# RustAudio/lewton

Hardware: NVIDIA H100
Metric: Msamples/s IMDCT+window+OLA, 2048-pt long blocks (higher is better)
Workload: dtype f32

## Files before the change

include/lewton_b200.h:

```cpp
#ifndef LEWTON_B200_H
#define LEWTON_B200_H

#include <stddef.h>
#include <stdint.h>

#ifdef __cplusplus
extern "C" {
#endif

#define LWB_ABI_VERSION 3
#define LWB_MAX_POSTS 65
#define LWB_MAX_CHANNELS 255
#define LWB_MAX_COUPLING 256
#define LWB_MAX_SUBMAPS 16
#define LWB_MAX_MODES 64

enum {
    LWB_OK = 0,
    LWB_ERR_BAD_FORMAT = 1,
    LWB_ERR_BUFFER = 2,
    LWB_ERR_MISMATCH = 3,
    LWB_ERR_INVALID = 4,
    LWB_ERR_CUDA = 5,
    LWB_ERR_NO_DEVICE = 6
};

typedef struct lwb_ctx lwb_ctx;
typedef struct lwb_setup lwb_setup;
typedef struct lwb_stream lwb_stream;

int lwb_abi_version(void);
int lwb_device_count(void);
int lwb_ctx_create(int device_ordinal, lwb_ctx **out);
void lwb_ctx_destroy(lwb_ctx *ctx);
int lwb_ctx_synchronize(lwb_ctx *ctx);
const char *lwb_last_error(const lwb_ctx *ctx);
void *lwb_ctx_cuda_stream(lwb_ctx *ctx);
uint64_t lwb_ctx_launch_count(const lwb_ctx *ctx);
enum { LWB_KERNEL_LONG = 0, LWB_KERNEL_LONG_S = 1, LWB_KERNEL_MID = 2, LWB_KERNEL_SHORT = 3, LWB_KERNEL_SHORT_G = 4,
       LWB_KERNEL_ROW_COPY = 5, LWB_KERNEL_CHAIN = 6, LWB_KERNEL_FLOOR1_SEGMENTS = 7, LWB_KERNEL_PROLOGUE_FUSED = 8,
       LWB_KERNEL_PROLOGUE = 9, LWB_KERNEL_IMDCT = 10, LWB_KERNEL_OVERLAP = 11, LWB_KERNEL_SAVE_STATE = 12,
       LWB_KERNEL_COUNT = 13 };
uint64_t lwb_ctx_kernel_launches(const lwb_ctx *ctx, int kernel_id);
void *lwb_host_alloc(size_t bytes);
void lwb_host_free(void *p);
int lwb_bind_host_to_device(int device_ordinal);
int lwb_device_alloc(lwb_ctx *ctx, size_t bytes, void **out);
void lwb_device_free(lwb_ctx *ctx, void *p);
int lwb_memcpy_h2d(lwb_ctx *ctx, void *dst_dev, const void *src_host, size_t bytes);
int lwb_memcpy_d2h(lwb_ctx *ctx, void *dst_host, const void *src_dev, size_t bytes);

int lwb_tables_generate(int blocksize_log2, float *a, float *b, float *c, float *window,
                        uint32_t *bitrev);

typedef struct lwb_tables_ref {
    const float *a, *b, *c;
    const float *window;
    const uint32_t *bitrev;
} lwb_tables_ref;

enum { LWB_FLOOR_TYPE_ZERO = 0, LWB_FLOOR_TYPE_ONE = 1 };
typedef struct lwb_floor_desc {
    uint8_t floor_type;
    uint8_t floor1_multiplier;
    uint8_t floor1_values;
    uint8_t reserved;
    uint32_t floor1_x_list[LWB_MAX_POSTS];
} lwb_floor_desc;

typedef struct lwb_mapping_desc {
    uint16_t coupling_steps;
    uint8_t submaps;
    uint8_t reserved;
    uint8_t magnitudes[LWB_MAX_COUPLING];
    uint8_t angles[LWB_MAX_COUPLING];
// ... 139 lines not shown
```

lewton_b200/_cabi.py:

```python
import ctypes as C
import os

_HERE = os.path.dirname(os.path.abspath(__file__))
SO_PATH = os.environ.get("LWB_LIB") or os.path.join(_HERE, "liblewton_b200.so")

MAX_POSTS, MAX_CHANNELS, MAX_COUPLING, MAX_SUBMAPS, MAX_MODES = 65, 255, 256, 16, 64
OK, ERR_BAD_FORMAT, ERR_BUFFER, ERR_MISMATCH, ERR_INVALID, ERR_CUDA, ERR_NO_DEVICE = range(7)
FLOOR_TYPE_ZERO, FLOOR_TYPE_ONE = 0, 1
FLOOR_UNUSED, FLOOR_ONE, FLOOR_DENSE = 0, 1, 2
OUT_F32_PLANAR, OUT_I16_PLANAR, OUT_F32_INTERLEAVED, OUT_I16_INTERLEAVED = 0, 1, 2, 3
ENTRY_SPECTRUM, ENTRY_RESIDUE, ENTRY_VQ = 0, 1, 2
MEM_HOST, MEM_DEVICE = 0, 1
KERNELS = ("k_long", "k_long_s", "k_mid", "k_short", "k_short_g", "k_row_copy", "k_chain", "k_floor1_segments",
           "k_prologue_fused", "k_prologue", "k_imdct", "k_overlap", "k_save_state")

vp, u8p, fp, u32p = C.c_void_p, C.POINTER(C.c_uint8), C.POINTER(C.c_float), C.POINTER(C.c_uint32)


class TablesRef(C.Structure):
    _fields_ = [("a", fp), ("b", fp), ("c", fp), ("window", fp), ("bitrev", u32p)]


class FloorDesc(C.Structure):
    _fields_ = [("floor_type", C.c_uint8), ("floor1_multiplier", C.c_uint8), ("floor1_values", C.c_uint8),
                ("reserved", C.c_uint8), ("floor1_x_list", C.c_uint32 * MAX_POSTS)]


class MappingDesc(C.Structure):
    _fields_ = [("coupling_steps", C.c_uint16), ("submaps", C.c_uint8), ("reserved", C.c_uint8),
                ("magnitudes", C.c_uint8 * MAX_COUPLING), ("angles", C.c_uint8 * MAX_COUPLING),
                ("mux", C.c_uint8 * (MAX_CHANNELS + 1)), ("submap_floors", C.c_uint8 * MAX_SUBMAPS)]


class ModeDesc(C.Structure):
    _fields_ = [("blockflag", C.c_uint8), ("mapping", C.c_uint8)]


class CodebookDesc(C.Structure):
    _fields_ = [("dimensions", C.c_uint16), ("reserved", C.c_uint16), ("entries", C.c_uint32), ("vq", fp)]


class ResidueDesc(C.Structure):
    _fields_ = [("residue_type", C.c_uint8), ("reserved", C.c_uint8 * 3), ("partition_size", C.c_uint32)]


class VqRun(C.Structure):
    _fields_ = [("pos", C.c_uint16), ("first", C.c_uint16), ("book", C.c_uint8), ("pass_kind", C.c_uint8), ("aux", C.c_uint8),
# ... 89 lines not shown
```

lewton_b200/csrc/host_objects.cuh:

```cuda
#pragma once

struct DevBuf {
    void *p = nullptr;
    size_t cap = 0;
};

struct Staging {
    void *h = nullptr;
    size_t cap = 0;
    cudaEvent_t ev = nullptr;
    bool pending = false;
};

struct CachedTables {
    DevTables dt;
    std::vector<float> a, b, c, w;
    std::vector<uint32_t> br;
    std::vector<void *> allocs;
};

struct lwb_ctx {
    int device = 0;
    int sm_count = 0;
    cudaStream_t stream = nullptr;
    cudaStream_t copy_in = nullptr, copy_out = nullptr;
    cudaEvent_t ev_in[64] = {}, ev_done[65] = {};
    DevBuf runs_buf[2];
    cudaEvent_t ev_desc[2] = {}, ev_kdone[2] = {};
    int runs_par = 0;
    uint32_t ticket_next = 0;
    uint64_t epoch = 0;
    uint64_t state_gen = 1;
    std::string err;
    uint64_t launches = 0;
    uint64_t kernel_launches[LWB_KERNEL_COUNT] = {};
    std::vector<PcmSpan> pcm_spans;
    std::vector<PcmCopy> pcm_copies;
    std::deque<CachedTables> tables;
    DevBuf coeffs, dense, pcm, spec, segtab, vqoff, vqrec, magic, x, desc, kinds, ys, chains, ticket, cdesc, cbytes;
    Staging stage[3];
    int stage_next = 0;
    void *h_desc = nullptr;
    size_t h_desc_cap = 0;
    size_t x_cap_elems = (size_t)64 << 20;
};

struct lwb_setup {
    lwb_ctx *ctx = nullptr;
    DevSetup host;
    DevSetup *d_setup = nullptr;
    std::vector<void *> allocs;
    uint8_t channels = 0, bs0 = 0, bs1 = 0;
    uint32_t n_modes = 0;
    uint32_t n_mappings = 0;
    std::vector<DevMapping> mappings;
};

struct MixRound { size_t r0, nr, s0, ns, c0, nc, x0, nx, g0, ng, flat, nm; };
struct RowCopy { const float *src; float *dst; uint32_t n4, pad; };
struct MixLaunch {
    char *db; size_t off_sr, off_cd, off_by, off_rc, off_sg;
    const float *pack, *spack, *w_short, *mpack; int ls, mid_kb; bool i16, residue; int out_format; unsigned warps; size_t smem; int n1max, wpc, np;
    const float *coeffs, *dense; const uint8_t *kinds; const uint32_t *ys; void *pcm;
};

struct FrontStages {
    const DevPacket *pk = nullptr;
    size_t n = 0;
    unsigned C = 0;
    bool fast = false;
    size_t smem_old = 0;
    int n2max = 0;
    uint64_t c_lo = 0;
    uint64_t r_lo = 0, r_hi = 0;
    bool dense = false;
};

struct lwb_plan {
    lwb_ctx *ctx = nullptr;
    lwb_chain *chains = nullptr;
    size_t n_chains = 0;
    lwb_batch_io io;
    bool captured = false;
    uint64_t gen = 0;
    FrontStages front;
    DevBuf runs, pro, mix;
    uint32_t n_groups = 0;
    const float *pack = nullptr;
    bool i16 = false;
    MixLaunch mix_launch;
    std::vector<MixRound> mix_rounds;
};

struct lwb_stream {
    lwb_ctx *ctx = nullptr;
    const lwb_setup *setup = nullptr;
    float *d_state = nullptr;
    bool has = false;
    uint32_t plen = 0;
    uint64_t busy_epoch = 0;
};

static inline void set_stream_state(lwb_stream *s, bool has, uint32_t plen)
{
    if (s->has != has || s->plen != plen) {
        s->has = has;
        s->plen = plen;
        s->ctx->state_gen++;
    }
}

static int fail(lwb_ctx *ctx, int code, const char *what, cudaError_t e = cudaSuccess)
{
    if (ctx) {
        ctx->err = what;
        if (e != cudaSuccess) {
            ctx->err += ": ";
            ctx->err += cudaGetErrorString(e);
        }
    }
    return code;
}

static inline void count_launch(lwb_ctx *ctx, int kernel_id)
{
    ctx->launches++;
    ctx->kernel_launches[kernel_id]++;
}

#define CU(ctx, call)                                                        \
    do {                                                                     \
        cudaError_t e__ = (call);                                            \
        if (e__ != cudaSuccess) return fail((ctx), LWB_ERR_CUDA, #call, e__); \
    } while (0)

static int ensure(lwb_ctx *ctx, DevBuf &b, size_t bytes)
{
    if (bytes <= b.cap) return LWB_OK;
    if (b.p) {
        CU(ctx, cudaStreamSynchronize(ctx->stream));
// ... 117 lines not shown
```

lewton_b200/csrc/kernel_long.cuh:

```cuda
#pragma once
#include <stdint.h>

#if defined(__CUDACC__)
#include <cuda_runtime.h>
#define LWB_HD __host__ __device__ __forceinline__
#else
#define LWB_HD inline
#endif

namespace lwb {

constexpr int kLongBs = 11;
constexpr int kLongN = 2048;
constexpr int kLongN2 = 1024;

struct alignas(16) LongRun {
    const float *in;
    void *out;
    float *state;
    uint32_t in_stride;
    uint32_t n_packets;
    uint8_t has_prev;
    uint8_t write_state;
    uint8_t dummy;
    uint8_t first_short;
    uint8_t last_short;
    uint8_t pad[3];
    float *state_out;
};
static_assert(sizeof(LongRun) == 48, "LongRun is copied by TMA in 16-byte units");

struct V { float x, y; };

#if defined(__CUDA_ARCH__)
__device__ __forceinline__ V vadd(V a, V b) { return V{__fadd_rn(a.x, b.x), __fadd_rn(a.y, b.y)}; }
__device__ __forceinline__ V vsub(V a, V b) { return V{__fsub_rn(a.x, b.x), __fsub_rn(a.y, b.y)}; }
__device__ __forceinline__ V vmul(V a, V b) { return V{__fmul_rn(a.x, b.x), __fmul_rn(a.y, b.y)}; }
__device__ __forceinline__ V vadd_p(V a, V b) { return V{__fadd_rn(a.x, b.x), __fadd_rn(a.y, b.y)}; }
__device__ __forceinline__ V vsub_p(V a, V b) { return V{__fsub_rn(a.x, b.x), __fsub_rn(a.y, b.y)}; }
__device__ __forceinline__ V vnsub_p(V a, V b) { return V{__fsub_rn(-a.x, b.x), __fsub_rn(-a.y, b.y)}; }
#else
inline V vadd(V a, V b) { return V{a.x + b.x, a.y + b.y}; }
inline V vsub(V a, V b) { return V{a.x - b.x, a.y - b.y}; }
inline V vmul(V a, V b) { return V{a.x * b.x, a.y * b.y}; }
inline V vadd_p(V a, V b) { return vadd(a, b); }
inline V vsub_p(V a, V b) { return vsub(a, b); }
inline V vnsub_p(V a, V b) { return V{-a.x - b.x, -a.y - b.y}; }
#endif

enum {
    P_S0W0 = 0, P_S0W1 = 8,
    P_S2W0 = 16, P_S2W1 = 20,
    P_L0W0 = 24, P_L0W1 = 26,
    P_L1W0 = 28, P_L1W1 = 29,
    P_A_END = 30,
    P_L2W0 = 30, P_L2W1 = 34,
    P_L3W0 = 38, P_L3W1 = 40,
    P_L4W0 = 42, P_L4W1 = 43,
    P_B_END = 44,
    P_A2 = 44,
// ... 315 lines not shown
constexpr int kLongWarps = LWB_LONG_WARPS;
constexpr int kLongRing = LWB_LONG_RING;
constexpr int kLongTileBytes = kLongN2 * 4;
constexpr int kLongStageBytes = kLongNB * kLongTileBytes;
constexpr size_t kLongSmemBytes = 2048 + (size_t)kLongWarps * (kLongRing + 1) * kLongStageBytes +
                                  (size_t)kLongPackFloats * 4 + kLongWarps * (kLongRing + 2) * 8 +
                                  kLongWarps * kLongNB * sizeof(LongRun) + 64;

__device__ __forceinline__ uint32_t smem_u32(const void *p) { return (uint32_t)__cvta_generic_to_shared(p); }

__device__ __forceinline__ void mbar_init(uint32_t bar, uint32_t count)
{
    asm volatile("mbarrier.init.shared::cta.b64 [%0], %1;" ::"r"(bar), "r"(count));
}
__device__ __forceinline__ void mbar_expect_tx(uint32_t bar, uint32_t bytes)
{
    asm volatile("mbarrier.arrive.expect_tx.shared::cta.b64 _, [%0], %1;" ::"r"(bar), "r"(bytes) : "memory");
}
__device__ __forceinline__ void mbar_wait(uint32_t bar, uint32_t parity)
{
    asm volatile(
        "{\n\t.reg .pred p;\n\t"
        "WAIT_%=:\n\t"
        "mbarrier.try_wait.parity.shared::cta.b64 p, [%0], %1, %2;\n\t"
        "@p bra DONE_%=;\n\t"
        "bra WAIT_%=;\n\t"
        "DONE_%=:\n\t}" ::"r"(bar), "r"(parity), "r"(200000u) : "memory");
}
__device__ __forceinline__ void tma_load_1d(uint32_t dst, const void *src, uint32_t bytes, uint32_t bar)
{
    asm volatile("cp.async.bulk.shared::cluster.global.mbarrier::complete_tx::bytes [%0], [%1], %2, [%3];"
                 ::"r"(dst), "l"(src), "r"(bytes), "r"(bar) : "memory");
}
__device__ __forceinline__ void fence_proxy_async()
{
    asm volatile("fence.proxy.async.shared::cta;" ::: "memory");
}
__device__ __forceinline__ void sts_eo(uint32_t addr, float e, float o)
{
    asm volatile("st.shared.f32 [%0], %1;\n\tst.shared.f32 [%0+2048], %2;" ::"r"(addr), "f"(e), "f"(o) : "memory");
}
__device__ __forceinline__ void lds_eo(uint32_t addr, float &e, float &o)
{
    asm volatile("ld.shared.f32 %0, [%2];\n\tld.shared.f32 %1, [%2+2048];" : "=f"(e), "=f"(o) : "r"(addr) : "memory");
}

#ifndef LWB_TW_REG0
#define LWB_TW_REG0 0
#endif
#ifndef LWB_TW_REG1
#define LWB_TW_REG1 (LWB_LONG_NB == 2 ? 0 : 53)
#endif
constexpr int kTwReg0 = LWB_TW_REG0;
constexpr int kTwReg1 = LWB_TW_REG1;
struct TwMix {
    const V *r;
    const V *lane_base;
    __device__ __forceinline__ V operator()(int slot) const
    {
        return (slot >= kTwReg0 && slot < kTwReg1) ? r[slot - kTwReg0] : lane_base[slot * 32];
    }
};

__device__ __forceinline__ uint32_t laneA(int lane, int half) { return 4u * (uint32_t)swz(elemA(lane, 0, half)); }
__device__ __forceinline__ uint32_t laneB(int lane) { return 4u * (uint32_t)swz(elemB(lane, 0, 0)); }
__device__ __forceinline__ uint32_t laneC(int lane, int half) { return 4u * (uint32_t)swz(elemC(lane, 0, half)); }
#define LWB_KA(j) (4u * (uint32_t)swz(64 * (j)))
#define LWB_KB(j, h) (4u * (uint32_t)swz(((h) << 6) | ((j) << 3)))
#define LWB_KC(j) (4u * (uint32_t)swz(j))

struct RunCur {
    const float *in;
    void *out;
    float *state;
    uint32_t in_stride;
    uint32_t flags;
};
__device__ __forceinline__ RunCur run_cur(const LongRun &r)
{
    return RunCur{r.in, r.out, r.state, r.in_stride,
                  (uint32_t)(r.has_prev ? 1u : 0u) | (r.write_state ? 2u : 0u) | (r.dummy ? 4u : 0u) |
                      (r.first_short ? 8u : 0u) | (r.last_short ? 16u : 0u)};
}
struct RunCurS : RunCur { float *state_out; };
__device__ __forceinline__ RunCurS run_cur_s(const LongRun &r)
{
    RunCurS c;
    static_cast<RunCur &>(c) = run_cur(r);
    c.flags |= r.first_short == 2 ? 32u : 0u;
    c.state_out = r.state_out ? r.state_out : r.state;
    return c;
}

__device__ __forceinline__ int16_t d_sample_i16(float v)
{
    short r;
    asm("cvt.rzi.s16.f32 %0, %1;" : "=h"(r) : "f"(__fmul_rn(v, 32768.0f)));
    return (int16_t)r;
}
__device__ __forceinline__ void st_pcm(float *p, float v) { __stcs(p, v); }
__device__ __forceinline__ void st_pcm(int16_t *p, float v) { __stcs(reinterpret_cast<short *>(p), (short)d_sample_i16(v)); }

template <int NB, bool FIRST, typename OutT, typename RC = RunCur>
__device__ __forceinline__ void out_stage(const TwMix &tw, int lane, const V O[NB][8], const V E[NB][8], V pe[NB][8],
                                          const RC cur[NB], OutT *out[NB], const float *s_state)
{
#pragma unroll
    for (int j = 0; j < 8; j++) {
        const int r64 = 64 * rev3(j);
        const bool nat = (j & 1);
        const V b0 = tw(P_B0 + j), b1 = tw(P_B1 + j);
        const V wlo = tw(P_WLO + j), whi = tw(P_WHI + j);
#pragma unroll
        for (int b = 0; b < NB; b++) {
            V plo = pe[b][j], phi = pe[b][j];
            bool emit = !(cur[b].flags & 4u);
            if (FIRST) {
                emit = emit && (cur[b].flags & 1u);
                if (cur[b].flags & 1u) {
                    const float *s_lo = s_state + b * kLongN2 + lane, *s_hi = s_state + b * kLongN2 + 63 - lane;
                    const float ax = nat ? s_lo[r64] : s_hi[r64], ay = nat ? s_hi[r64] : s_lo[r64];
                    const float bx = nat ? s_hi[960 - r64] : s_lo[960 - r64];
                    const float by = nat ? s_lo[960 - r64] : s_hi[960 - r64];
                    plo = V{ax, ay};
                    phi = V{bx, by};
                }
            }
            V lo, hi, pev;
            step8_ola(b0, b1, wlo, whi, O[b][j], E[b][j], plo, phi, lo, hi, pev);
            pe[b][j] = pev;
            if (emit) {
                OutT *o_lo = out[b] + lane, *o_hi = out[b] + 63 - lane;
                if (nat) {
                    st_pcm(o_lo + r64, lo.x); st_pcm(o_hi + r64, lo.y);
                    st_pcm(o_hi + 960 - r64, hi.x); st_pcm(o_lo + 960 - r64, hi.y);
                } else {
                    st_pcm(o_hi + r64, lo.x); st_pcm(o_lo + r64, lo.y);
                    st_pcm(o_lo + 960 - r64, hi.x); st_pcm(o_hi + 960 - r64, hi.y);
                }
            }
        }
    }
}

__device__ __forceinline__ float lds_f32(uint32_t addr)
{
    float v;
    asm volatile("ld.shared.f32 %0, [%1];" : "=f"(v) : "r"(addr) : "memory");
    return v;
}

template <int NB, typename OutT, typename RC = RunCur, bool EXPORT = false, int LS = 0>
__device__ __forceinline__ void out_first_short(const TwMix &tw, int lane, const V O[NB][8], const V E[NB][8], V pe[NB][8],
                                                const RC cur[NB], OutT *out[NB], const float *s_state,
                                                const float *__restrict__ w, int ls_arg, uint32_t w_s = 0)
{
    const int ls = LS ? LS : ls_arg;
    const int pl = kLongN2 - 2 * ls;
// ... 77 lines not shown
    const uint32_t bar_state = bars_s + 8 * kLongRing, bar_desc = bars_s + 8 * (kLongRing + 1);
    const uint32_t state_s = smem_u32(s_state), next_s = smem_u32(s_next);
    const uint32_t lA0 = laneA(lane, 0), lA1 = laneA(lane, 1);
    const uint32_t lB = laneB(lane);
    const uint32_t lC0 = laneC(lane, 0), lC1 = laneC(lane, 1);
    uint32_t phase_bits = 0;
    uint32_t slot_i = 0;

    uint32_t lc = 0;
    uint32_t nx_idx = 0;
    uint32_t nx_stage = 0;
    uint32_t nx_lc = 0, nx_npk = 0;
    uint32_t nx_state_issued = 0;
    uint32_t desc_parity = 0;
    RunCur cur[NB];
    uint32_t npk;

    auto issue_stage = [&](uint32_t stage, const LongRun *r, uint32_t pkt) {
        const uint32_t bar = bars_s + 8 * stage;
        mbar_expect_tx(bar, kLongStageBytes);
#pragma unroll
        for (int b = 0; b < NB; b++)
            tma_load_1d(tiles_s + stage * kLongStageBytes + b * kLongTileBytes,
                        r[b].in + (size_t)pkt * r[b].in_stride, kLongTileBytes, bar);
    };
    auto issue_stage_cur = [&](uint32_t stage, uint32_t pkt) {
        const uint32_t bar = bars_s + 8 * stage;
        mbar_expect_tx(bar, kLongStageBytes);
#pragma unroll
        for (int b = 0; b < NB; b++)
            tma_load_1d(tiles_s + stage * kLongStageBytes + b * kLongTileBytes,
                        cur[b].in + (size_t)pkt * cur[b].in_stride, kLongTileBytes, bar);
    };
    auto issue_state = [&](const float *const st[NB], const uint32_t has[NB]) {
        uint32_t bytes = 0;
#pragma unroll
        for (int b = 0; b < NB; b++) bytes += has[b] ? kLongTileBytes : 0;
        mbar_expect_tx(bar_state, bytes);
#pragma unroll
        for (int b = 0; b < NB; b++)
            if (has[b]) tma_load_1d(state_s + b * kLongTileBytes, st[b], kLongTileBytes, bar_state);
    };

    {
        uint32_t idx = 0;
        if (lane == 0) idx = atomicAdd(ticket, 1u);
        idx = __shfl_sync(0xffffffffu, idx, 0);
        if (idx >= n_groups) return;
#pragma unroll
        for (int b = 0; b < NB; b++) cur[b] = run_cur(runs[idx * NB + b]);
        npk = runs[idx * NB].n_packets;
        if (lane == 0) {
            fence_proxy_async();
            const float *st[NB];
            uint32_t has[NB];
#pragma unroll
            for (int b = 0; b < NB; b++) { st[b] = cur[b].state; has[b] = cur[b].flags & 1u; }
            issue_state(st, has);
            for (; lc < (uint32_t)kLongRing && lc < npk; lc++) issue_stage_cur(lc, lc);
            nx_idx = atomicAdd(ticket, 1u);
        }
    }

    for (;;) {
        V pe[NB][8];
#pragma unroll
        for (int b = 0; b < NB; b++)
#pragma unroll
            for (int j = 0; j < 8; j++) pe[b][j] = V{0.f, 0.f};
        OutT *out[NB];
#pragma unroll
        for (int b = 0; b < NB; b++) out[b] = static_cast<OutT *>(cur[b].out);

        for (uint32_t p = 0; p < npk; p++) {
            const uint32_t stage_s = tiles_s + slot_i * kLongStageBytes;
            mbar_wait(bars_s + 8 * slot_i, (phase_bits >> slot_i) & 1u);
            phase_bits ^= 1u << slot_i;

            V O[NB][8], E[NB][8];
            {
                const float *tp[NB];
#pragma unroll
                for (int b = 0; b < NB; b++) tp[b] = tiles + (slot_i * NB + b) * kLongN2;
                phase_a<NB>(tp, lane, tw, O, E);
            }
            __syncwarp();
#pragma unroll
            for (int b = 0; b < NB; b++) {
                const uint32_t t = stage_s + b * kLongTileBytes;
                const uint32_t a0 = t + lA0, a1 = t + lA1;
#pragma unroll
// ... 49 lines not shown
                uint32_t ahead = lc - (p + 1) + nx_lc;
                if (ahead < (uint32_t)kLongRing) {
                    uint32_t tgt = slot_i + 1 + ahead;
                    if (tgt >= (uint32_t)kLongRing) tgt -= kLongRing;
                    if (lc < npk) {
                        fence_proxy_async();
                        issue_stage_cur(tgt, lc);
                        lc++;
                    } else {
                        if (nx_stage == 1) {
                            mbar_wait(bar_desc, desc_parity);
                            desc_parity ^= 1u;
                            nx_stage = 2;
                            nx_npk = s_next[0].n_packets;
                            nx_lc = 0;
                        }
                        if (nx_stage == 2 && nx_lc < nx_npk) {
                            fence_proxy_async();
                            issue_stage(tgt, s_next, nx_lc);
                            nx_lc++;
                        }
                    }
                }
            }
            phase_c_fft<NB>(tw, O, E);
            if (p > 0) {
                out_stage<NB, false, OutT>(tw, lane, O, E, pe, cur, out, s_state);
            } else {
                mbar_wait(bar_state, (phase_bits >> 30) & 1u);
                phase_bits ^= 1u << 30;
                if (NB == 1 && (cur[0].flags & 8u))
                    out_first_short<NB, OutT>(tw, lane, O, E, pe, cur, out, s_state, w_short, ls);
                else
                    out_stage<NB, true, OutT>(tw, lane, O, E, pe, cur, out, s_state);
                __syncwarp();
            }
#pragma unroll
            for (int b = 0; b < NB; b++)
                if (p > 0 || (cur[b].flags & 1u)) out[b] += (p == 0 && (cur[b].flags & 8u)) ? kLongN2 - ls : kLongN2;
            if (lane == 0 && nx_stage == 2 && !nx_state_issued) {
                const float *st[NB];
                uint32_t has[NB];
#pragma unroll
                for (int b = 0; b < NB; b++) { st[b] = s_next[b].state; has[b] = s_next[b].has_prev; }
                fence_proxy_async();
                issue_state(st, has);
                nx_state_issued = 1;
            }
            slot_i = (slot_i + 1 == (uint32_t)kLongRing) ? 0 : slot_i + 1;
        }
#pragma unroll
        for (int b = 0; b < NB; b++) {
            if ((cur[b].flags & 16u)) {
                const bool emitted = (npk > 1 || (cur[b].flags & 1u)) && !(cur[b].flags & 4u);
                const bool keep = (cur[b].flags & 6u) == 2u;
#pragma unroll
                for (int j = 0; j < 8; j++) {
                    const int r64 = 64 * rev3(j);
#pragma unroll
                    for (int h = 0; h < 2; h++) {
                        const float v = ((j & 1) != 0) == (h == 0) ? pe[b][j].x : pe[b][j].y;
                        const int m = r64 + (h ? 63 - lane : lane);
                        if (m < ls) {
                            if (emitted) st_pcm(out[b] + m, v);
                        } else if (keep && m < kLongN2 - ls) {
                            cur[b].state[m - ls] = v;
                            cur[b].state[kLongN2 - 1 - ls - m] = v;
                        }
                    }
                }
            } else if ((cur[b].flags & 6u) == 2u) {
                float *s_lo = cur[b].state + lane, *s_hi = cur[b].state + 63 - lane;
#pragma unroll
                for (int j = 0; j < 8; j++) {
                    const int r64 = 64 * rev3(j);
                    const float vx = (j & 1) ? pe[b][j].x : pe[b][j].y, vy = (j & 1) ? pe[b][j].y : pe[b][j].x;
                    s_lo[r64] = vx; s_hi[r64] = vy;
                    s_hi[960 - r64] = vx; s_lo[960 - r64] = vy;
                }
            }
        }
        uint32_t st_ = 0, nlc = 0;
        if (lane == 0) {
            if (nx_stage == 0) {
                if (nx_idx < n_groups) {
                    fence_proxy_async();
                    mbar_expect_tx(bar_desc, NB * (uint32_t)sizeof(LongRun));
                    tma_load_1d(next_s, runs + (size_t)nx_idx * NB, NB * (uint32_t)sizeof(LongRun), bar_desc);
                    nx_stage = 1;
                } else {
                    nx_stage = 3;
                }
            }
            if (nx_stage == 1) {
                mbar_wait(bar_desc, desc_parity);
                desc_parity ^= 1u;
                nx_stage = 2;
                nx_npk = s_next[0].n_packets;
                nx_lc = 0;
            }
            if (nx_stage == 2 && !nx_state_issued) {
                const float *st[NB];
                uint32_t has[NB];
#pragma unroll
                for (int b = 0; b < NB; b++) { st[b] = s_next[b].state; has[b] = s_next[b].has_prev; }
                fence_proxy_async();
                issue_state(st, has);
            }
            st_ = nx_stage;
            nlc = nx_lc;
        }
        st_ = __shfl_sync(0xffffffffu, st_, 0);
        nlc = __shfl_sync(0xffffffffu, nlc, 0);
        if (st_ != 2) break;
        __syncwarp();
#pragma unroll
        for (int b = 0; b < NB; b++) cur[b] = run_cur(s_next[b]);
        npk = s_next[0].n_packets;
        __syncwarp();
        lc = nlc;
        nx_stage = 0; nx_lc = 0; nx_npk = 0; nx_state_issued = 0;
        if (lane == 0) {
            fence_proxy_async();
            for (uint32_t k = lc; k < (uint32_t)kLongRing && k < npk; k++) {
                issue_stage_cur((slot_i + k) % kLongRing, k);
                lc = k + 1;
            }
            nx_idx = atomicAdd(ticket, 1u);
        }
    }
}

__device__ __forceinline__ void cp_async16(uint32_t dst, const void *src)
{
    asm volatile("cp.async.cg.shared.global [%0], [%1], 16;" ::"r"(dst), "l"(src) : "memory");
}
__device__ __forceinline__ void cp_async_commit() { asm volatile("cp.async.commit_group;" ::: "memory"); }
template <int N>
__device__ __forceinline__ void cp_async_wait() { asm volatile("cp.async.wait_group %0;" ::"n"(N) : "memory"); }

constexpr int kLongLs256 = (kLongN - 256) / 4;
constexpr int kLongFetch = 3;
constexpr int kLongDescSlots = kLongFetch + kLongRing + 3;
constexpr int kLongSlopeMax = 512;
constexpr size_t kLongSmemBytesS = 2048 + (size_t)kLongWarps * (kLongRing + 1) * kLongTileBytes + (size_t)kLongPackFloats * 4 +
                                   kLongWarps * (kLongRing + 2) * 8 + (size_t)kLongWarps * kLongDescSlots * sizeof(LongRun) +
                                   kLongSlopeMax * sizeof(float) + 64;

template <typename OutT, int LS>
__global__ void __launch_bounds__(kLongWarps * 32, 1)
// ... 257 lines not shown
```

lewton_b200/csrc/lwb_api.cu:

```cuda
#include <cuda_runtime.h>
#include <sched.h>
#include <sys/syscall.h>
#include <unistd.h>

#include <algorithm>
#include <cctype>
#include <cstdio>
#include <cstdlib>
#include <cstring>
#include <deque>
#include <new>
#include <string>
#include <vector>

#include "kernel_long.cuh"
#include "kernel_short.cuh"
#include "kernel_mid.cuh"
#include "kernels_generic.cuh"
#include "kernel_chain.cuh"
#include "kernel_prologue.cuh"
#include "lwb_common.h"
#include "pcm_copy_plan.h"

namespace lwb {
// ... 30 lines not shown
    if (!ctx) return LWB_ERR_BUFFER;
    ctx->device = device;
    ctx->sm_count = prop.multiProcessorCount;
    if (cudaSetDevice(device) != cudaSuccess ||
        cudaStreamCreateWithFlags(&ctx->stream, cudaStreamNonBlocking) != cudaSuccess ||
        cudaStreamCreateWithFlags(&ctx->copy_in, cudaStreamNonBlocking) != cudaSuccess ||
        cudaStreamCreateWithFlags(&ctx->copy_out, cudaStreamNonBlocking) != cudaSuccess) {
        delete ctx;
        return LWB_ERR_CUDA;
    }
    if (create_pipeline_objects(ctx)) {
        lwb_ctx_destroy(ctx);
        return LWB_ERR_CUDA;
    }
    if (const char *e = getenv("LWB_SCRATCH_MB")) {
        long mb = atol(e);
        if (mb >= 1) ctx->x_cap_elems = (size_t)mb << 18;
    }
    long_kernel_configure();
    short_kernel_configure();
    mid_kernel_configure();
    prologue_kernel_configure();
    *out = ctx;
    return LWB_OK;
}

extern "C" void lwb_ctx_destroy(lwb_ctx *ctx)
{
    if (!ctx) return;
    cudaSetDevice(ctx->device);
    cudaStreamSynchronize(ctx->stream);
    for (DevBuf *b : {&ctx->coeffs, &ctx->dense, &ctx->pcm, &ctx->spec, &ctx->segtab, &ctx->vqoff, &ctx->vqrec, &ctx->magic, &ctx->x, &ctx->desc,
                      &ctx->kinds, &ctx->ys, &ctx->chains, &ctx->ticket, &ctx->runs_buf[0], &ctx->runs_buf[1],
                      &ctx->cdesc, &ctx->cbytes})
        if (b->p) cudaFree(b->p);
    for (CachedTables &ct : ctx->tables)
        for (void *p : ct.allocs) cudaFree(p);
    if (ctx->h_desc) cudaFreeHost(ctx->h_desc);
    for (Staging &st : ctx->stage) {
        if (st.h) cudaFreeHost(st.h);
        if (st.ev) cudaEventDestroy(st.ev);
    }
    for (cudaEvent_t e : ctx->ev_in) if (e) cudaEventDestroy(e);
    for (cudaEvent_t e : ctx->ev_done) if (e) cudaEventDestroy(e);
    for (int k = 0; k < 2; k++) {
        if (ctx->ev_desc[k]) cudaEventDestroy(ctx->ev_desc[k]);
        if (ctx->ev_kdone[k]) cudaEventDestroy(ctx->ev_kdone[k]);
    }
    cudaStreamDestroy(ctx->stream);
    cudaStreamDestroy(ctx->copy_in);
    cudaStreamDestroy(ctx->copy_out);
    delete ctx;
}

extern "C" int lwb_ctx_synchronize(lwb_ctx *ctx)
{
    if (!ctx) return LWB_ERR_INVALID;
    CU(ctx, cudaSetDevice(ctx->device));
    CU(ctx, cudaStreamSynchronize(ctx->stream));
    return LWB_OK;
}

extern "C" const char *lwb_last_error(const lwb_ctx *ctx) { return ctx ? ctx->err.c_str() : "no context"; }
extern "C" void *lwb_ctx_cuda_stream(lwb_ctx *ctx) { return ctx ? (void *)ctx->stream : nullptr; }
extern "C" uint64_t lwb_ctx_launch_count(const lwb_ctx *ctx) { return ctx ? ctx->launches : 0; }
extern "C" uint64_t lwb_ctx_kernel_launches(const lwb_ctx *ctx, int kernel_id)
{
// ... 291 lines not shown
    if (e != cudaSuccess) {
        delete s;
        return fail(ctx, LWB_ERR_CUDA, "stream_open: cudaMalloc", e);
    }
    *out = s;
    return LWB_OK;
}

extern "C" void lwb_stream_destroy(lwb_stream *s)
{
    if (!s) return;
    cudaSetDevice(s->ctx->device);
    cudaStreamSynchronize(s->ctx->stream);
    cudaFree(s->d_state);
    delete s;
}

extern "C" int lwb_stream_reset(lwb_stream *s)
{
    if (!s) return LWB_ERR_INVALID;
    set_stream_state(s, false, 0);
    return LWB_OK;
}
extern "C" int lwb_stream_is_empty(const lwb_stream *s) { return (!s || !s->has) ? 1 : 0; }
extern "C" uint32_t lwb_stream_state_len(const lwb_stream *s) { return (s && s->has) ? s->plen : 0; }

extern "C" int lwb_stream_clone(const lwb_stream *s, lwb_stream **out)
{
    if (!s || !out) return LWB_ERR_INVALID;
    int rc = lwb_stream_open(s->ctx, s->setup, out);
    if (rc) return rc;
    (*out)->has = s->has;
    (*out)->plen = s->plen;
    lwb_ctx *ctx = s->ctx;
    CU(ctx, cudaMemcpyAsync((*out)->d_state, s->d_state,
                            s->setup->channels * state_stride(s->setup) * sizeof(float),
                            cudaMemcpyDeviceToDevice, ctx->stream));
    return LWB_OK;
}

extern "C" int lwb_stream_export_state(lwb_stream *s, float *out)
{
    if (!s || !out) return LWB_ERR_INVALID;
    if (!s->has) return LWB_OK;
    lwb_ctx *ctx = s->ctx;
    CU(ctx, cudaSetDevice(ctx->device));
    CU(ctx, cudaMemcpy2DAsync(out, s->plen * sizeof(float), s->d_state, state_stride(s->setup) * sizeof(float),
                              s->plen * sizeof(float), s->setup->channels, cudaMemcpyDeviceToHost, ctx->stream));
    CU(ctx, cudaStreamSynchronize(ctx->stream));
    return LWB_OK;
}

extern "C" int lwb_stream_import_state(lwb_stream *s, const float *data, uint32_t len)
{
    if (!s || (!data && len)) return LWB_ERR_INVALID;
    if (len > state_stride(s->setup)) return LWB_ERR_BUFFER;
    lwb_ctx *ctx = s->ctx;
    CU(ctx, cudaSetDevice(ctx->device));
    if (len) {
        CU(ctx, cudaMemcpy2DAsync(s->d_state, state_stride(s->setup) * sizeof(float), data, len * sizeof(float),
                                  len * sizeof(float), s->setup->channels, cudaMemcpyHostToDevice, ctx->stream));
        CU(ctx, cudaStreamSynchronize(ctx->stream));
    }
    s->ctx->state_gen++;
    s->has = true;
    s->plen = len;
    return LWB_OK;
}

extern "C" int lwb_decoded_sample_count(const lwb_setup *su, uint8_t mode, int prev_flag, int next_flag,
                                        uint32_t *n_samples)
{
    if (!su || !n_samples) return LWB_ERR_INVALID;
    Geom g;
    int rc = geometry(su, mode, prev_flag, next_flag, &g);
    if (rc) return rc;
    *n_samples = g.rs - g.ls;
    return LWB_OK;
}

#include "path_generic.cuh"
#include "path_long.cuh"
#include "path_chain.cuh"
#include "path_mixed.cuh"
#include "path_mid.cuh"

using BatchPath = int (*)(lwb_ctx *, lwb_chain *, size_t, const lwb_batch_io *, uint64_t, bool *, lwb_plan *);
static const BatchPath kBatchPaths[] = {
    [](lwb_ctx *ctx, lwb_chain *chains, size_t n, const lwb_batch_io *io, uint64_t epoch, bool *handled, lwb_plan *plan) {
        return try_long(ctx, chains, n, io, epoch, handled, plan);
    },
    try_long_residue, try_mid, try_mixed, try_chain};
constexpr size_t kNumBatchPaths = sizeof(kBatchPaths) / sizeof(kBatchPaths[0]);

static size_t first_batch_path()
{
    const char *fg = getenv("LWB_FORCE_GENERIC");
    if (!fg) return 0;
    return std::strcmp(fg, "1") == 0 ? kNumBatchPaths : kNumBatchPaths - 1;
}

static int decode_chains_impl(lwb_ctx *ctx, lwb_chain *chains, size_t n_chains, const lwb_batch_io *io, lwb_plan *prepared)
{
    if (!ctx || (!chains && n_chains) || !io) return LWB_ERR_INVALID;
    if (io->entry != LWB_ENTRY_SPECTRUM && io->entry != LWB_ENTRY_RESIDUE && io->entry != LWB_ENTRY_VQ) return fail(ctx, LWB_ERR_INVALID, "bad entry");
    if (io->memory != LWB_MEM_HOST && io->memory != LWB_MEM_DEVICE) return fail(ctx, LWB_ERR_INVALID, "bad memory space");
    if (io->out_format < 0 || io->out_format > LWB_OUT_I16_INTERLEAVED) return fail(ctx, LWB_ERR_INVALID, "bad out_format");
    if (n_chains == 0) return LWB_OK;
    if ((!io->coeffs && io->entry != LWB_ENTRY_VQ) || !io->pcm) return fail(ctx, LWB_ERR_INVALID, "null arena");
    if (io->entry == LWB_ENTRY_VQ && (!io->vq_runs || !io->vq_run_offsets || !io->vq_entries || !io->vq_entry_offsets || !io->floor_kind))
        return fail(ctx, LWB_ERR_INVALID, "VQ entry needs vq_runs, vq_entries, their offsets and floor_kind");
    CU(ctx, cudaSetDevice(ctx->device));
    const uint64_t epoch = ++ctx->epoch;
    if (prepared) {
        prepared->captured = false;
        prepared->mix_rounds.clear();
    }
    for (size_t k = first_batch_path(); k < kNumBatchPaths; k++) {
        bool handled = false;
        const int rc = kBatchPaths[k](ctx, chains, n_chains, io, epoch, &handled, prepared);
        if (rc || handled) return rc;
    }
    const bool vq = io->entry == LWB_ENTRY_VQ;
    const bool residue = io->entry != LWB_ENTRY_SPECTRUM;
    const bool planar = is_planar(io->out_format);
    std::vector<PlanChain> plan(n_chains);
    uint64_t c_lo = ~0ull, c_hi = 0, o_lo = ~0ull, o_hi = 0, r_lo = ~0ull, r_hi = 0;
    int uniform_c = -1;
    bool need_dense = false;
    for (size_t i = 0; i < n_chains; i++) {
        lwb_chain *c = &chains[i];
        if (!c->stream || c->stream->ctx != ctx || (c->n_packets && !c->mode_numbers))
            return fail(ctx, LWB_ERR_INVALID, "chain: bad stream or mode list");
        if (c->stream->busy_epoch == epoch) return fail(ctx, LWB_ERR_INVALID, "a stream appears in two chains of one batch");
        c->stream->busy_epoch = epoch;
        const int C = c->stream->setup->channels;
        if (residue) {
            if (uniform_c < 0) uniform_c = C;
            if (uniform_c != C) return fail(ctx, LWB_ERR_INVALID, "residue batches need one channel count");
            if (!io->floor_kind) return fail(ctx, LWB_ERR_INVALID, "residue entry needs floor_kind");
        }
        plan_chain(c, &plan[i]);
        PlanChain &pc = plan[i];
        if (pc.pk.empty()) continue;
        const PlanPacket &last = pc.pk.back();
        c_lo = std::min(c_lo, c->coeff_offset);
        c_hi = std::max(c_hi, last.coeff_off + (uint64_t)C * (last.g.n >> 1));
        const uint64_t ext = planar ? (uint64_t)(C - 1) * c->out_stride + c->n_samples : (uint64_t)c->n_samples * C;
        if (planar && c->out_stride < c->n_samples) return fail(ctx, LWB_ERR_BUFFER, "chain: out_stride smaller than the samples produced");
        o_lo = std::min(o_lo, c->out_offset);
        o_hi = std::max(o_hi, c->out_offset + ext);
        if (residue) {
            r_lo = std::min(r_lo, c->packet_index);
            r_hi = std::max<uint64_t>(r_hi, c->packet_index + pc.pk.size());
            int krc = scan_floor_kinds(ctx, io, c->packet_index * C, (c->packet_index + pc.pk.size()) * C, &need_dense);
// ... 222 lines not shown
```

lewton_b200/csrc/path_long.cuh:

```cuda
#pragma once

struct LongItem {
    lwb_chain *c;
    uint32_t P;
    bool has_prev;
};

static int acquire_staging(lwb_ctx *ctx, size_t bytes, Staging **out)
{
    Staging &st = ctx->stage[ctx->stage_next];
    ctx->stage_next = (ctx->stage_next + 1) % 3;
    if (!st.ev) CU(ctx, cudaEventCreateWithFlags(&st.ev, cudaEventDisableTiming));
    if (st.pending) {
        CU(ctx, cudaEventSynchronize(st.ev));
        st.pending = false;
    }
    if (st.cap < bytes) {
        if (st.h) cudaFreeHost(st.h);
        st.h = nullptr;
        st.cap = 0;
        CU(ctx, cudaHostAlloc(&st.h, bytes * 2 + 4096, cudaHostAllocDefault));
        st.cap = bytes * 2 + 4096;
    }
    *out = &st;
    return LWB_OK;
}

static void long_runs_of(const LongItem &it, size_t cuts, const float *coeffs, uint64_t coeff_base, char *pcm,
                         uint64_t pcm_base, size_t esz, LongRun *&w)
{
    const lwb_stream *s = it.c->stream;
    const lwb_setup *su = s->setup;
    const unsigned C = su->channels;
    const size_t P = it.P;
    for (unsigned ch = 0; ch < C; ch++) {
        const float *in0 = coeffs + (it.c->coeff_offset - coeff_base) + (size_t)ch * kLongN2;
        char *out0 = pcm + ((it.c->out_offset - pcm_base) + (size_t)ch * it.c->out_stride) * esz;
        for (size_t k = 0; k < cuts; k++) {
            const size_t p0 = P * k / cuts, p1 = P * (k + 1) / cuts;
            LongRun &r = *w++;
            std::memset(&r, 0, sizeof(r));
            r.in_stride = (uint32_t)(C * kLongN2);
            r.state = s->d_state + (size_t)ch * state_stride(su);
            r.write_state = (k + 1 == cuts);
            if (k == 0) {
                r.in = in0;
                r.n_packets = (uint32_t)(p1 - p0);
                r.has_prev = it.has_prev;
                r.out = out0;
            } else {
                r.in = in0 + (p0 - 1) * (size_t)r.in_stride;
                r.n_packets = (uint32_t)(p1 - p0 + 1);
                r.has_prev = 0;
                r.out = out0 + (size_t)(p0 - (it.has_prev ? 0 : 1)) * kLongN2 * esz;
            }
        }
    }
}

static bool batch_is_uniform_long(lwb_ctx *ctx, const lwb_chain *chains, size_t n_chains, const lwb_batch_io *io)
{
    if (io->out_format != LWB_OUT_F32_PLANAR && io->out_format != LWB_OUT_I16_PLANAR) return false;
    const float *pack = nullptr;
    for (size_t i = 0; i < n_chains; i++) {
        const lwb_chain *c = &chains[i];
        if (!c->stream || c->stream->ctx != ctx || (c->n_packets && !c->mode_numbers)) return false;
        const lwb_stream *s = c->stream;
        const lwb_setup *su = s->setup;
        if (su->bs1 != kLongBs || !su->host.tab[1].pack) return false;
        if (pack && pack != su->host.tab[1].pack) return false;
        pack = su->host.tab[1].pack;
        if ((c->out_offset & 3) || (c->out_stride & 3) || (c->coeff_offset & 3) || !device_arenas_aligned(io)) return false;
        if (s->has && s->plen != (uint32_t)kLongN2) return false;
        for (uint32_t k = 0; k < c->n_packets; k++) {
            const uint8_t m = c->mode_numbers[k];
            if (m >= su->n_modes || !su->host.mode_blockflag[m]) return false;
            if (c->prev_window_flags && !c->prev_window_flags[k]) return false;
            if (c->next_window_flags && !c->next_window_flags[k]) return false;
        }
    }
    return true;
// ... 159 lines not shown
    CU(ctx, cudaEventRecord(ctx->ev_desc[par], ds));
    CU(ctx, cudaEventRecord(st->ev, ds));
    st->pending = true;
    CU(ctx, cudaStreamWaitEvent(ctx->stream, ctx->ev_desc[par], 0));
    for (size_t k = 0; k < cplan.size(); k++) {
        const ChunkPlan &cp = cplan[k];
        if (in_host) {
            CU(ctx, cudaMemcpyAsync((float *)ctx->coeffs.p + (cp.kc_lo - cbase), io->coeffs + cp.kc_lo,
                                    (size_t)(cp.kc_hi - cp.kc_lo) * 4, cudaMemcpyHostToDevice, ctx->copy_in));
            CU(ctx, cudaEventRecord(ctx->ev_in[k], ctx->copy_in));
            CU(ctx, cudaStreamWaitEvent(ctx->stream, ctx->ev_in[k], 0));
        }
        if ((rc = launch_long(ctx, d_runs_base + cp.r0, (uint32_t)(cp.nr / kLongNB), pack, i16))) return rc;
        if (host && cp.ko_hi > cp.ko_lo) {
            const size_t evk = slice.active ? (size_t)slice.ev_slot : k;
            CU(ctx, cudaEventRecord(ctx->ev_done[evk], ctx->stream));
            CU(ctx, cudaStreamWaitEvent(ctx->copy_out, ctx->ev_done[evk], 0));
            if ((rc = copy_pcm_to_host(ctx, io, chains, cp.i0, cp.i1, ctx->pcm.p, obase, ctx->copy_out))) return rc;
        }
    }
    CU(ctx, cudaEventRecord(ctx->ev_kdone[par], ctx->stream));
    if (capture && cplan.size() == 1) {
        plan->captured = true;
        plan->gen = gen_at_entry;
        plan->n_groups = (uint32_t)(cplan[0].nr / kLongNB);
        plan->pack = pack;
        plan->i16 = i16;
    }
    if (host && !slice.active) {
        CU(ctx, cudaStreamSynchronize(ctx->copy_out));
        CU(ctx, cudaStreamSynchronize(ctx->stream));
    }
    for (auto &it : items)
        if (it.P) set_stream_state(it.c->stream, true, kLongN2);
    return LWB_OK;
}

static int try_long_residue(lwb_ctx *ctx, lwb_chain *chains, size_t n_chains, const lwb_batch_io *io, uint64_t epoch, bool *handled,
                            lwb_plan *plan)
{
    *handled = false;
    if (io->entry == LWB_ENTRY_SPECTRUM) return LWB_OK;
    if (!batch_is_uniform_long(ctx, chains, n_chains, io)) return LWB_OK;
    const bool vq = io->entry == LWB_ENTRY_VQ;
    if (!io->floor_kind) return fail(ctx, LWB_ERR_INVALID, "residue entry needs floor_kind");
    unsigned C = 0;
    size_t n_pk = 0;
    uint64_t c_lo = ~0ull, c_hi = 0, r_lo = ~0ull, r_hi = 0;
    bool need_dense = false;
    int rc;
    for (size_t i = 0; i < n_chains; i++) {
        const lwb_chain *c = &chains[i];
        const unsigned cc = c->stream->setup->channels;
        if (!C) C = cc;
        if (C != cc) return fail(ctx, LWB_ERR_INVALID, "residue batches need one channel count");
        if (!c->n_packets) continue;
        n_pk += c->n_packets;
        c_lo = std::min(c_lo, c->coeff_offset);
        c_hi = std::max(c_hi, c->coeff_offset + (uint64_t)c->n_packets * C * kLongN2);
        r_lo = std::min(r_lo, c->packet_index);
        r_hi = std::max<uint64_t>(r_hi, c->packet_index + c->n_packets);
        if ((rc = scan_floor_kinds(ctx, io, c->packet_index * C, (c->packet_index + c->n_packets) * C, &need_dense))) return rc;
    }
    if (need_dense && !io->dense_floor) return fail(ctx, LWB_ERR_INVALID, "dense_floor missing");
    for (size_t i = 0; i < n_chains; i++) {
        lwb_stream *s = chains[i].stream;
        if (s->busy_epoch == epoch) return fail(ctx, LWB_ERR_INVALID, "a stream appears in two chains of one batch");
// ... 146 lines not shown
```

Measured before the change: 316,500.

## Store only half of palindromic overlap state and mirror lazily on demand

The long-block kernel now writes only the first half of the symmetric overlap-add state row and reads back only that half on the next batch, rebuilding the mirrored half in registers. This halves state write and read traffic. A separate mirror kernel fills in the full rows when a different path needs them, and export mirrors on the host. State stores and loads also carry an L2 evict_last cache hint. The cost is extra flag handling and a possible extra kernel launch when paths switch.

```diff
diff --git a/include/lewton_b200.h b/include/lewton_b200.h
--- a/include/lewton_b200.h
+++ b/include/lewton_b200.h
@@ -40,7 +40,7 @@
 enum { LWB_KERNEL_LONG = 0, LWB_KERNEL_LONG_S = 1, LWB_KERNEL_MID = 2, LWB_KERNEL_SHORT = 3, LWB_KERNEL_SHORT_G = 4,
        LWB_KERNEL_ROW_COPY = 5, LWB_KERNEL_CHAIN = 6, LWB_KERNEL_FLOOR1_SEGMENTS = 7, LWB_KERNEL_PROLOGUE_FUSED = 8,
        LWB_KERNEL_PROLOGUE = 9, LWB_KERNEL_IMDCT = 10, LWB_KERNEL_OVERLAP = 11, LWB_KERNEL_SAVE_STATE = 12,
-       LWB_KERNEL_COUNT = 13 };
+       LWB_KERNEL_STATE_MIRROR = 13, LWB_KERNEL_COUNT = 14 };
 uint64_t lwb_ctx_kernel_launches(const lwb_ctx *ctx, int kernel_id);
 void *lwb_host_alloc(size_t bytes);
 void lwb_host_free(void *p);
diff --git a/lewton_b200/_cabi.py b/lewton_b200/_cabi.py
--- a/lewton_b200/_cabi.py
+++ b/lewton_b200/_cabi.py
@@ -12,7 +12,7 @@
 ENTRY_SPECTRUM, ENTRY_RESIDUE, ENTRY_VQ = 0, 1, 2
 MEM_HOST, MEM_DEVICE = 0, 1
 KERNELS = ("k_long", "k_long_s", "k_mid", "k_short", "k_short_g", "k_row_copy", "k_chain", "k_floor1_segments",
-           "k_prologue_fused", "k_prologue", "k_imdct", "k_overlap", "k_save_state")
+           "k_prologue_fused", "k_prologue", "k_imdct", "k_overlap", "k_save_state", "k_state_mirror")
 
 vp, u8p, fp, u32p = C.c_void_p, C.POINTER(C.c_uint8), C.POINTER(C.c_float), C.POINTER(C.c_uint32)
 
diff --git a/lewton_b200/csrc/host_objects.cuh b/lewton_b200/csrc/host_objects.cuh
--- a/lewton_b200/csrc/host_objects.cuh
+++ b/lewton_b200/csrc/host_objects.cuh
@@ -37,7 +37,7 @@
     std::vector<PcmSpan> pcm_spans;
     std::vector<PcmCopy> pcm_copies;
     std::deque<CachedTables> tables;
-    DevBuf coeffs, dense, pcm, spec, segtab, vqoff, vqrec, magic, x, desc, kinds, ys, chains, ticket, cdesc, cbytes;
+    DevBuf coeffs, dense, pcm, spec, segtab, vqoff, vqrec, magic, x, desc, kinds, ys, chains, ticket, cdesc, cbytes, mirror_rows;
     Staging stage[3];
     int stage_next = 0;
     void *h_desc = nullptr;
@@ -98,14 +98,16 @@
     float *d_state = nullptr;
     bool has = false;
     uint32_t plen = 0;
+    bool mirrored = false;
     uint64_t busy_epoch = 0;
 };
 
-static inline void set_stream_state(lwb_stream *s, bool has, uint32_t plen)
-{
-    if (s->has != has || s->plen != plen) {
+static inline void set_stream_state(lwb_stream *s, bool has, uint32_t plen, bool mirrored = false)
+{
+    if (s->has != has || s->plen != plen || s->mirrored != mirrored) {
         s->has = has;
         s->plen = plen;
+        s->mirrored = mirrored;
         s->ctx->state_gen++;
     }
 }
diff --git a/lewton_b200/csrc/kernel_long.cuh b/lewton_b200/csrc/kernel_long.cuh
--- a/lewton_b200/csrc/kernel_long.cuh
+++ b/lewton_b200/csrc/kernel_long.cuh
@@ -25,7 +25,8 @@
     uint8_t dummy;
     uint8_t first_short;
     uint8_t last_short;
-    uint8_t pad[3];
+    uint8_t mirror;
+    uint8_t pad[2];
     float *state_out;
 };
 static_assert(sizeof(LongRun) == 48, "LongRun is copied by TMA in 16-byte units");
@@ -407,6 +408,21 @@
     asm volatile("cp.async.bulk.shared::cluster.global.mbarrier::complete_tx::bytes [%0], [%1], %2, [%3];"
                  ::"r"(dst), "l"(src), "r"(bytes), "r"(bar) : "memory");
 }
+__device__ __forceinline__ uint64_t l2_policy_last()
+{
+    uint64_t p;
+    asm volatile("createpolicy.fractional.L2::evict_last.b64 %0, 1.0;" : "=l"(p));
+    return p;
+}
+__device__ __forceinline__ void tma_load_1d_hint(uint32_t dst, const void *src, uint32_t bytes, uint32_t bar, uint64_t pol)
+{
+    asm volatile("cp.async.bulk.shared::cluster.global.mbarrier::complete_tx::bytes.L2::cache_hint [%0], [%1], %2, [%3], %4;"
+                 ::"r"(dst), "l"(src), "r"(bytes), "r"(bar), "l"(pol) : "memory");
+}
+__device__ __forceinline__ void st_last(float *p, float v, uint64_t pol)
+{
+    asm volatile("st.global.L2::cache_hint.f32 [%0], %1, %2;" ::"l"(p), "f"(v), "l"(pol) : "memory");
+}
 __device__ __forceinline__ void fence_proxy_async()
 {
     asm volatile("fence.proxy.async.shared::cta;" ::: "memory");
@@ -457,6 +473,16 @@
                   (uint32_t)(r.has_prev ? 1u : 0u) | (r.write_state ? 2u : 0u) | (r.dummy ? 4u : 0u) |
                       (r.first_short ? 8u : 0u) | (r.last_short ? 16u : 0u)};
 }
+__device__ __forceinline__ RunCur run_cur_long(const LongRun &r)
+{
+    RunCur c = run_cur(r);
+    c.flags |= (uint32_t)(r.mirror & 3u) << 6;
+    return c;
+}
+__device__ __forceinline__ uint32_t state_read_bytes(uint32_t has_prev, uint32_t mirror)
+{
+    return !has_prev ? 0u : (mirror & 1u) ? (uint32_t)kLongN2 * 2u : (uint32_t)kLongN2 * 4u;
+}
 struct RunCurS : RunCur { float *state_out; };
 __device__ __forceinline__ RunCurS run_cur_s(const LongRun &r)
 {
@@ -476,7 +502,7 @@
 __device__ __forceinline__ void st_pcm(float *p, float v) { __stcs(p, v); }
 __device__ __forceinline__ void st_pcm(int16_t *p, float v) { __stcs(reinterpret_cast<short *>(p), (short)d_sample_i16(v)); }
 
-template <int NB, bool FIRST, typename OutT, typename RC = RunCur>
+template <int NB, bool FIRST, typename OutT, typename RC = RunCur, bool MIRROR = false>
 __device__ __forceinline__ void out_stage(const TwMix &tw, int lane, const V O[NB][8], const V E[NB][8], V pe[NB][8],
                                           const RC cur[NB], OutT *out[NB], const float *s_state)
 {
@@ -497,8 +523,9 @@
                     const float ax = nat ? s_lo[r64] : s_hi[r64], ay = nat ? s_hi[r64] : s_lo[r64];
                     const float bx = nat ? s_hi[960 - r64] : s_lo[960 - r64];
                     const float by = nat ? s_lo[960 - r64] : s_hi[960 - r64];
+                    const bool half = MIRROR && (cur[b].flags & 64u);
                     plo = V{ax, ay};
-                    phi = V{bx, by};
+                    phi = V{half ? ax : bx, half ? ay : by};
                 }
             }
             V lo, hi, pev;
@@ -642,14 +669,14 @@
             tma_load_1d(tiles_s + stage * kLongStageBytes + b * kLongTileBytes,
                         cur[b].in + (size_t)pkt * cur[b].in_stride, kLongTileBytes, bar);
     };
-    auto issue_state = [&](const float *const st[NB], const uint32_t has[NB]) {
+    auto issue_state = [&](const float *const st[NB], const uint32_t rd[NB]) {
         uint32_t bytes = 0;
 #pragma unroll
-        for (int b = 0; b < NB; b++) bytes += has[b] ? kLongTileBytes : 0;
+        for (int b = 0; b < NB; b++) bytes += rd[b];
         mbar_expect_tx(bar_state, bytes);
 #pragma unroll
         for (int b = 0; b < NB; b++)
-            if (has[b]) tma_load_1d(state_s + b * kLongTileBytes, st[b], kLongTileBytes, bar_state);
+            if (rd[b]) tma_load_1d_hint(state_s + b * kLongTileBytes, st[b], rd[b], bar_state, l2_policy_last());
     };
 
     {
@@ -658,15 +685,15 @@
         idx = __shfl_sync(0xffffffffu, idx, 0);
         if (idx >= n_groups) return;
 #pragma unroll
-        for (int b = 0; b < NB; b++) cur[b] = run_cur(runs[idx * NB + b]);
+        for (int b = 0; b < NB; b++) cur[b] = run_cur_long(runs[idx * NB + b]);
         npk = runs[idx * NB].n_packets;
         if (lane == 0) {
             fence_proxy_async();
             const float *st[NB];
-            uint32_t has[NB];
-#pragma unroll
-            for (int b = 0; b < NB; b++) { st[b] = cur[b].state; has[b] = cur[b].flags & 1u; }
-            issue_state(st, has);
+            uint32_t rd[NB];
+#pragma unroll
+            for (int b = 0; b < NB; b++) { st[b] = cur[b].state; rd[b] = state_read_bytes(cur[b].flags & 1u, cur[b].flags >> 6); }
+            issue_state(st, rd);
             for (; lc < (uint32_t)kLongRing && lc < npk; lc++) issue_stage_cur(lc, lc);
             nx_idx = atomicAdd(ticket, 1u);
         }
@@ -782,7 +809,7 @@
                 if (NB == 1 && (cur[0].flags & 8u))
                     out_first_short<NB, OutT>(tw, lane, O, E, pe, cur, out, s_state, w_short, ls);
                 else
-                    out_stage<NB, true, OutT>(tw, lane, O, E, pe, cur, out, s_state);
+                    out_stage<NB, true, OutT, RunCur, true>(tw, lane, O, E, pe, cur, out, s_state);
                 __syncwarp();
             }
 #pragma unroll
@@ -790,11 +817,11 @@
                 if (p > 0 || (cur[b].flags & 1u)) out[b] += (p == 0 && (cur[b].flags & 8u)) ? kLongN2 - ls : kLongN2;
             if (lane == 0 && nx_stage == 2 && !nx_state_issued) {
                 const float *st[NB];
-                uint32_t has[NB];
-#pragma unroll
-                for (int b = 0; b < NB; b++) { st[b] = s_next[b].state; has[b] = s_next[b].has_prev; }
+                uint32_t rd[NB];
+#pragma unroll
+                for (int b = 0; b < NB; b++) { st[b] = s_next[b].state; rd[b] = state_read_bytes(s_next[b].has_prev, s_next[b].mirror); }
                 fence_proxy_async();
-                issue_state(st, has);
+                issue_state(st, rd);
                 nx_state_issued = 1;
             }
             slot_i = (slot_i + 1 == (uint32_t)kLongRing) ? 0 : slot_i + 1;
@@ -821,12 +848,14 @@
                 }
             } else if ((cur[b].flags & 6u) == 2u) {
                 float *s_lo = cur[b].state + lane, *s_hi = cur[b].state + 63 - lane;
+                const bool full = !(cur[b].flags & 128u);
+                const uint64_t pol = l2_policy_last();
 #pragma unroll
                 for (int j = 0; j < 8; j++) {
                     const int r64 = 64 * rev3(j);
                     const float vx = (j & 1) ? pe[b][j].x : pe[b][j].y, vy = (j & 1) ? pe[b][j].y : pe[b][j].x;
-                    s_lo[r64] = vx; s_hi[r64] = vy;
-                    s_hi[960 - r64] = vx; s_lo[960 - r64] = vy;
+                    st_last(s_lo + r64, vx, pol); st_last(s_hi + r64, vy, pol);
+                    if (full) { s_hi[960 - r64] = vx; s_lo[960 - r64] = vy; }
                 }
             }
         }
@@ -851,11 +880,11 @@
             }
             if (nx_stage == 2 && !nx_state_issued) {
                 const float *st[NB];
-                uint32_t has[NB];
-#pragma unroll
-                for (int b = 0; b < NB; b++) { st[b] = s_next[b].state; has[b] = s_next[b].has_prev; }
+                uint32_t rd[NB];
+#pragma unroll
+                for (int b = 0; b < NB; b++) { st[b] = s_next[b].state; rd[b] = state_read_bytes(s_next[b].has_prev, s_next[b].mirror); }
                 fence_proxy_async();
-                issue_state(st, has);
+                issue_state(st, rd);
             }
             st_ = nx_stage;
             nlc = nx_lc;
@@ -865,7 +894,7 @@
         if (st_ != 2) break;
         __syncwarp();
 #pragma unroll
-        for (int b = 0; b < NB; b++) cur[b] = run_cur(s_next[b]);
+        for (int b = 0; b < NB; b++) cur[b] = run_cur_long(s_next[b]);
         npk = s_next[0].n_packets;
         __syncwarp();
         lc = nlc;
diff --git a/lewton_b200/csrc/lwb_api.cu b/lewton_b200/csrc/lwb_api.cu
--- a/lewton_b200/csrc/lwb_api.cu
+++ b/lewton_b200/csrc/lwb_api.cu
@@ -86,7 +86,7 @@
     cudaStreamSynchronize(ctx->stream);
     for (DevBuf *b : {&ctx->coeffs, &ctx->dense, &ctx->pcm, &ctx->spec, &ctx->segtab, &ctx->vqoff, &ctx->vqrec, &ctx->magic, &ctx->x, &ctx->desc,
                       &ctx->kinds, &ctx->ys, &ctx->chains, &ctx->ticket, &ctx->runs_buf[0], &ctx->runs_buf[1],
-                      &ctx->cdesc, &ctx->cbytes})
+                      &ctx->cdesc, &ctx->cbytes, &ctx->mirror_rows})
         if (b->p) cudaFree(b->p);
     for (CachedTables &ct : ctx->tables)
         for (void *p : ct.allocs) cudaFree(p);
@@ -444,6 +444,7 @@
     if (rc) return rc;
     (*out)->has = s->has;
     (*out)->plen = s->plen;
+    (*out)->mirrored = s->mirrored;
     lwb_ctx *ctx = s->ctx;
     CU(ctx, cudaMemcpyAsync((*out)->d_state, s->d_state,
                             s->setup->channels * state_stride(s->setup) * sizeof(float),
@@ -457,9 +458,13 @@
     if (!s->has) return LWB_OK;
     lwb_ctx *ctx = s->ctx;
     CU(ctx, cudaSetDevice(ctx->device));
+    const uint32_t n = s->mirrored ? s->plen / 2 : s->plen;
     CU(ctx, cudaMemcpy2DAsync(out, s->plen * sizeof(float), s->d_state, state_stride(s->setup) * sizeof(float),
-                              s->plen * sizeof(float), s->setup->channels, cudaMemcpyDeviceToHost, ctx->stream));
+                              n * sizeof(float), s->setup->channels, cudaMemcpyDeviceToHost, ctx->stream));
     CU(ctx, cudaStreamSynchronize(ctx->stream));
+    if (s->mirrored)
+        for (unsigned ch = 0; ch < s->setup->channels; ch++)
+            for (uint32_t m = 0; m < n; m++) out[(size_t)ch * s->plen + s->plen - 1 - m] = out[(size_t)ch * s->plen + m];
     return LWB_OK;
 }
 
@@ -477,6 +482,7 @@
     s->ctx->state_gen++;
     s->has = true;
     s->plen = len;
+    s->mirrored = false;
     return LWB_OK;
 }
 
@@ -504,6 +510,7 @@
     },
     try_long_residue, try_mid, try_mixed, try_chain};
 constexpr size_t kNumBatchPaths = sizeof(kBatchPaths) / sizeof(kBatchPaths[0]);
+constexpr size_t kFirstFullRowPath = 2;
 
 static size_t first_batch_path()
 {
@@ -528,11 +535,20 @@
         prepared->captured = false;
         prepared->mix_rounds.clear();
     }
+    auto complete_batch_rows = [&]() {
+        std::vector<lwb_stream *> mirrored;
+        for (size_t i = 0; i < n_chains; i++)
+            if (chains[i].stream && chains[i].stream->ctx == ctx && chains[i].stream->mirrored) mirrored.push_back(chains[i].stream);
+        return complete_mirrored_rows(ctx, mirrored);
+    };
     for (size_t k = first_batch_path(); k < kNumBatchPaths; k++) {
+        if (k >= kFirstFullRowPath)
+            if (int rc = complete_batch_rows()) return rc;
         bool handled = false;
         const int rc = kBatchPaths[k](ctx, chains, n_chains, io, epoch, &handled, prepared);
         if (rc || handled) return rc;
     }
+    if (int rc = complete_batch_rows()) return rc;
     const bool vq = io->entry == LWB_ENTRY_VQ;
     const bool residue = io->entry != LWB_ENTRY_SPECTRUM;
     const bool planar = is_planar(io->out_format);
diff --git a/lewton_b200/csrc/path_long.cuh b/lewton_b200/csrc/path_long.cuh
--- a/lewton_b200/csrc/path_long.cuh
+++ b/lewton_b200/csrc/path_long.cuh
@@ -23,6 +23,41 @@
         st.cap = bytes * 2 + 4096;
     }
     *out = &st;
+    return LWB_OK;
+}
+
+__global__ void k_state_mirror(float *const *__restrict__ rows)
+{
+    float4 *row = reinterpret_cast<float4 *>(rows[blockIdx.x]);
+    const int t = threadIdx.x;
+    const float4 v = row[t];
+    row[kLongN2 / 4 - 1 - t] = make_float4(v.w, v.z, v.y, v.x);
+}
+
+static int complete_mirrored_rows(lwb_ctx *ctx, std::vector<lwb_stream *> &streams)
+{
+    std::sort(streams.begin(), streams.end());
+    streams.erase(std::unique(streams.begin(), streams.end()), streams.end());
+    size_t n_rows = 0;
+    for (const lwb_stream *s : streams) n_rows += s->mirrored ? s->setup->channels : 0;
+    if (!n_rows) return LWB_OK;
+    int rc;
+    Staging *st;
+    if ((rc = acquire_staging(ctx, n_rows * sizeof(float *), &st))) return rc;
+    if ((rc = ensure(ctx, ctx->mirror_rows, n_rows * sizeof(float *)))) return rc;
+    float **h = (float **)st->h;
+    size_t k = 0;
+    for (const lwb_stream *s : streams)
+        if (s->mirrored)
+            for (unsigned ch = 0; ch < s->setup->channels; ch++) h[k++] = s->d_state + (size_t)ch * state_stride(s->setup);
+    CU(ctx, cudaMemcpyAsync(ctx->mirror_rows.p, h, n_rows * sizeof(float *), cudaMemcpyHostToDevice, ctx->stream));
+    CU(ctx, cudaEventRecord(st->ev, ctx->stream));
+    st->pending = true;
+    if ((rc = launch(ctx, LWB_KERNEL_STATE_MIRROR, k_state_mirror, dim3((unsigned)n_rows), dim3(kLongN2 / 8), 0,
+                     (float *const *)ctx->mirror_rows.p)))
+        return rc;
+    for (lwb_stream *s : streams)
+        if (s->mirrored) set_stream_state(s, s->has, s->plen);
     return LWB_OK;
 }
 
@@ -43,10 +78,12 @@
             r.in_stride = (uint32_t)(C * kLongN2);
             r.state = s->d_state + (size_t)ch * state_stride(su);
             r.write_state = (k + 1 == cuts);
+            r.mirror = r.write_state ? 2 : 0;
             if (k == 0) {
                 r.in = in0;
                 r.n_packets = (uint32_t)(p1 - p0);
                 r.has_prev = it.has_prev;
+                r.mirror |= (it.has_prev && s->mirrored) ? 1 : 0;
                 r.out = out0;
             } else {
                 r.in = in0 + (p0 - 1) * (size_t)r.in_stride;
@@ -272,7 +309,7 @@
         CU(ctx, cudaStreamSynchronize(ctx->stream));
     }
     for (auto &it : items)
-        if (it.P) set_stream_state(it.c->stream, true, kLongN2);
+        if (it.P) set_stream_state(it.c->stream, true, kLongN2, true);
     return LWB_OK;
 }
 
```

Result: faster. 323,500, median of 6 (+2.2%).
